# alexranaldi/CWSL_DIGI

Hardware: AMD Instinct MI355X
Metric: IQ Msamples/s demod+sync per GPU; concurrent FT8 slots at real-time; % HBM roofline (higher is better)
Workload: dtype f32

## Files before the change

cwsl_digi_amd/csrc/sync_host.inc:

```
namespace {

int sync_ensure_shared(cwslg_ctx *c)
{
    if (c->sync_shared.d_tables) return CWSLG_OK;
    constexpr double pi = 3.14159265358979323846;
    auto w = [&](int k, double n) { return make_float2((float)std::cos(2.0 * pi * k / n), (float)(-std::sin(2.0 * pi * k / n))); };
    auto half = [](float2 v) { return make_float2(0.5f * v.x, 0.5f * v.y); };
    auto same = [](float a, float b) { return std::memcmp(&a, &b, 4) == 0; };
    for (int k = 1; k <= 4; ++k)
        if (!same(w(k, 9.0).x, small_wr<9>(k)) || !same(w(k, 9.0).y, small_wi<9>(k)))
            return fail(c, CWSLG_ERR_HIP, "sync tables: W_9^%d computed on this host differs from the kernels' constants", k);
    for (int k = 1; k <= 2; ++k)
        if (!same(w(k, 5.0).x, w5_r(k)) || !same(w(k, 5.0).y, w5_i(k)))
            return fail(c, CWSLG_ERR_HIP, "sync tables: W_5^%d computed on this host differs from the kernels' constants", k);
    if (!same((float)(-std::sin(2.0 * pi / 3.0)), W3_S))
        return fail(c, CWSLG_ERR_HIP, "sync tables: sin(2 pi / 3) computed on this host differs from the kernels' constant");
    std::vector<float2> t;
    t.reserve(1920 + 64 + 1921 + 1152 + 1153);
    const float fac = 1.0f / 300.0f;
    for (int k = 0; k < 1920; ++k) { const float2 v = (k == 0) ? make_float2(1.f, 0.f) : w(k, 1920.0); t.push_back(make_float2(fac * v.x, fac * v.y)); }
    for (int k = 0; k < 64; ++k) t.push_back(w(k, 128.0));
    for (int k = 0; k <= 1920; ++k) t.push_back(half(k == 0 ? make_float2(1.f, 0.f) : w(k, 3840.0)));
    t[1920] = make_float2(1.f, 0.f); t[1920 + 32] = make_float2(0.f, -1.f);
    const size_t ft8_count = t.size();
    for (int k = 0; k < 1152; ++k) t.push_back(w(k, 1152.0));
    for (int k = 0; k <= 1152; ++k) t.push_back(half(k == 0 ? make_float2(1.f, 0.f) : w(k, 2304.0)));
    t[ft8_count] = make_float2(1.f, 0.f);
    HIPCHK(c, hipMalloc(&c->sync_shared.d_tables, t.size() * sizeof(float2)));
    HIPCHK(c, hipMemcpy(c->sync_shared.d_tables, t.data(), t.size() * sizeof(float2), hipMemcpyHostToDevice));
    c->sync_shared.t.w1920 = c->sync_shared.d_tables;
    c->sync_shared.t.w128 = c->sync_shared.d_tables + 1920;
    c->sync_shared.t.w3840 = c->sync_shared.d_tables + 1920 + 64;
    c->sync_shared.t.win = nullptr;
    float2 *t4 = c->sync_shared.d_tables + ft8_count;
    c->sync_shared.t4.w1920 = t4;
    c->sync_shared.t4.w128 = c->sync_shared.t.w128;
    c->sync_shared.t4.w3840 = t4 + 1152;
    std::vector<float> win(FT4_NFFT1);
    for (int i = 0; i < FT4_NFFT1; ++i)
        win[i] = (float)(0.3635819 - 0.4891775 * std::cos(2.0 * pi * i / 2304.0) + 0.1365995 * std::cos(4.0 * pi * i / 2304.0)
                         - 0.0106411 * std::cos(6.0 * pi * i / 2304.0));
    HIPCHK(c, hipMalloc(&c->sync_shared.d_win, win.size() * sizeof(float)));
    HIPCHK(c, hipMemcpy(c->sync_shared.d_win, win.data(), win.size() * sizeof(float), hipMemcpyHostToDevice));
    c->sync_shared.t4.win = c->sync_shared.d_win;
    return CWSLG_OK;
}

int ft4c_ensure_tables(cwslg_ctx *c)
{
    if (c->sync_shared.d_ft4c) return CWSLG_OK;
    constexpr double pi = 3.14159265358979323846;
    auto mk = [](double co, double si) { return make_float2((float)co, (float)si); };
    std::vector<float2> t;
    const size_t o567 = 0, on2 = o567 + F4C_NA, o2n = on2 + F4C_N2, o64 = o2n + F4C_N2 + 1, o63 = o64 + 32, o4032 = o63 + 63,
                 ocs = o4032 + F4C_NP, otw = ocs + 256, total = otw + 33 * 64;
    t.resize(total);
    for (int k = 0; k < F4C_NA; ++k) t[o567 + k] = mk(std::cos(2.0 * pi * k / 567.0), -std::sin(2.0 * pi * k / 567.0));
    for (int k = 0; k < F4C_N2; ++k) t[on2 + k] = mk(std::cos(2.0 * pi * k / 36288.0), -std::sin(2.0 * pi * k / 36288.0));
    for (int k = 0; k <= F4C_N2; ++k) t[o2n + k] = mk(std::cos(2.0 * pi * k / 72576.0), -std::sin(2.0 * pi * k / 72576.0));
    for (int k = 0; k < 32; ++k) t[o64 + k] = mk(std::cos(2.0 * pi * k / 64.0), -std::sin(2.0 * pi * k / 64.0));
    for (int k = 0; k < 63; ++k) t[o63 + k] = mk(std::cos(2.0 * pi * k / 63.0), -std::sin(2.0 * pi * k / 63.0));
    for (int k = 0; k < F4C_NP; ++k) t[o4032 + k] = mk(std::cos(2.0 * pi * k / 4032.0), -std::sin(2.0 * pi * k / 4032.0));
    t[o567] = t[on2] = t[o2n] = t[o64] = t[o63] = t[o4032] = mk(1.0, 0.0);
    t[o64 + 16] = mk(0.0, -1.0);
    {
        std::vector<float2> flat(t.begin() + on2, t.begin() + on2 + F4C_N2);
        for (int cc = 0; cc < F4C_NA; ++cc) for (int b = 0; b < 64; ++b) t[on2 + (size_t)cc * 64 + b] = flat[(size_t)b * cc];
        flat.assign(t.begin() + o4032, t.begin() + o4032 + F4C_NP);
        for (int cc = 0; cc < 63; ++cc) for (int b = 0; b < 64; ++b) t[o4032 + (size_t)cc * 64 + b] = flat[(size_t)b * cc];
    }
    static const int icos4[4][4] = {{0, 1, 3, 2}, {1, 0, 2, 3}, {2, 3, 1, 0}, {3, 2, 0, 1}};
    for (int b = 0; b < 4; ++b)
        for (int sy = 0; sy < 4; ++sy)
            for (int j = 0; j < 16; ++j) {
                const int p = (2 * icos4[b][sy] * j) % 32;
                float2 v = mk(std::cos(2.0 * pi * p / 32.0), std::sin(2.0 * pi * p / 32.0));
                if (p == 0) v = mk(1.0, 0.0);
                if (p == 8) v = mk(0.0, 1.0);
                if (p == 16) v = mk(-1.0, 0.0);
                if (p == 24) v = mk(0.0, -1.0);
                t[ocs + 64 * b + 16 * sy + j] = v;
            }
    for (int d = -16; d <= 16; ++d)
        for (int k = 0; k < 64; ++k) {
            const double a = 2.0 * pi * (double)d * (double)(k + 1) * 36.0 / 12000.0;
            t[otw + (d + 16) * 64 + k] = (d == 0) ? mk(1.0, 0.0) : mk(std::cos(a), std::sin(a));
        }
    std::vector<float> win(F4C_KHI - F4C_KLO + 1);
    for (int k = F4C_KLO; k <= F4C_KHI; ++k) {
        const int i = k + 126;
        double wv = 1.0;
        if (i < 63) wv = 0.5 * (1.0 + std::cos(pi * (double)(62 - i) / 63.0));
        else if (i >= 567) wv = 0.5 * (1.0 + std::cos(pi * (double)(i - 567) / 63.0));
        win[k - F4C_KLO] = (float)wv;
    }
    HIPCHK(c, hipMalloc(&c->sync_shared.d_ft4c, t.size() * sizeof(float2)));
    HIPCHK(c, hipMemcpy(c->sync_shared.d_ft4c, t.data(), t.size() * sizeof(float2), hipMemcpyHostToDevice));
    HIPCHK(c, hipMalloc(&c->sync_shared.d_ft4c_win, win.size() * sizeof(float)));
    HIPCHK(c, hipMemcpy(c->sync_shared.d_ft4c_win, win.data(), win.size() * sizeof(float), hipMemcpyHostToDevice));
    const float2 *b = c->sync_shared.d_ft4c;
    c->ft4_tables = Ft4Tables{b + o567, b + on2, b + o2n, b + o64, b + o63, b + o4032, b + ocs, b + otw, c->sync_shared.d_ft4c_win};
    return CWSLG_OK;
}

int ft4c_ensure_channel(cwslg_ctx *c, Channel &ch)
{
// ... 389 lines not shown
```

cwsl_digi_amd/csrc/sync_kernels.hpp:

```cpp
#pragma once
#include <hip/hip_runtime.h>
#include <stdint.h>

namespace cwslg {

constexpr int FT8_NSPS = 1920, FT8_NSTEP = 480, FT8_NHSYM = 372, FT8_NH1 = 1920, FT8_JZ = 62, FT8_NMAX = 180000;
constexpr int FT4_NFFT1 = 2304, FT4_NSTEP = 576, FT4_NHSYM = 122, FT4_NH1 = 1152, FT4_NMAX = 72576;
constexpr int FT4_ROW = 1168;
constexpr int SYNC_BAND = 32;
constexpr int SYNC_MAXCAND_CAP = 600;
constexpr int SYNC_MAXPRE = 1000;

struct SyncConfig {
    bool enabled = false;
    float syncmin = 1.5f;
    float syncmin_ft4 = 1.2f;
    bool ft4_coherent = true;
    int max_cand = 200;
    int order = 0;
    int f_lo_hz = 200, f_hi_hz = 3000;
    int ia = 64, ib = 960, nbins = 976;
};

struct SyncTables {
// ... 109 lines not shown
constexpr float W3_S = -0x1.bb67aep-1f;

template <int HALF>
__device__ __forceinline__ void stage1_pfa15(const float2 (&z)[8], float2 (*s_y)[SY_PITCH], const float2 *tw, int b)
{
    constexpr int KP = HALF ? 2 : 1;
    float2 Ya[3], Yb[3];
    {
        constexpr float w1r = w5r_at((1 * KP) % 5), w1i = w5i_at((1 * KP) % 5), w2r = w5r_at((2 * KP) % 5), w2i = w5i_at((2 * KP) % 5);
        float P = z[3].x * w1r, Q = z[3].y * w1i, R = z[3].x * w1i, S = z[3].y * w1r;
        P = __builtin_fmaf(z[6].x, w2r, P); Q = __builtin_fmaf(z[6].y, w2i, Q); R = __builtin_fmaf(z[6].x, w2i, R); S = __builtin_fmaf(z[6].y, w2r, S);
        Ya[0] = make_float2(z[0].x + (P - Q), z[0].y + (R + S));
        Yb[0] = make_float2(z[0].x + (P + Q), z[0].y + (S - R));
    }
    {
        constexpr float wr = w5r_at((4 * KP) % 5), wi = w5i_at((4 * KP) % 5);
        const float P = z[2].x * wr, Q = z[2].y * wi, R = z[2].x * wi, S = z[2].y * wr;
        Ya[1] = make_float2(z[5].x + (P - Q), z[5].y + (R + S));
        Yb[1] = make_float2(z[5].x + (P + Q), z[5].y + (S - R));
    }
    {
        constexpr float w1r = w5r_at((2 * KP) % 5), w1i = w5i_at((2 * KP) % 5), w2r = w5r_at((3 * KP) % 5), w2i = w5i_at((3 * KP) % 5),
                        w3r = w5r_at((4 * KP) % 5), w3i = w5i_at((4 * KP) % 5);
        float P = z[1].x * w1r, Q = z[1].y * w1i, R = z[1].x * w1i, S = z[1].y * w1r;
        P = __builtin_fmaf(z[4].x, w2r, P); Q = __builtin_fmaf(z[4].y, w2i, Q); R = __builtin_fmaf(z[4].x, w2i, R); S = __builtin_fmaf(z[4].y, w2r, S);
        P = __builtin_fmaf(z[7].x, w3r, P); Q = __builtin_fmaf(z[7].y, w3i, Q); R = __builtin_fmaf(z[7].x, w3i, R); S = __builtin_fmaf(z[7].y, w3r, S);
        Ya[2] = make_float2(P - Q, R + S);
        Yb[2] = make_float2(P + Q, S - R);
    }
    int n = 0;
    auto three = [&](const float2 y0, const float2 y1, const float2 y2, int k2) {
        const float2 x0 = make_float2((y0.x + y1.x) + y2.x, (y0.y + y1.y) + y2.y);
        const float2 t = make_float2(y1.x + y2.x, y1.y + y2.y), d = make_float2(y1.x - y2.x, y1.y - y2.y);
        const float2 m = make_float2(__builtin_fmaf(t.x, -0.5f, y0.x), __builtin_fmaf(t.y, -0.5f, y0.y));
        const float2 x1 = make_float2(__builtin_fmaf(-W3_S, d.y, m.x), __builtin_fmaf(W3_S, d.x, m.y));
        const float2 x2 = make_float2(__builtin_fmaf(W3_S, d.y, m.x), __builtin_fmaf(-W3_S, d.x, m.y));
        const int c0 = pfa15_c(0, k2), c1 = pfa15_c(1, k2), c2 = pfa15_c(2, k2);
        if (c0 == 0) s_y[0][b] = make_float2(x0.x * (1.0f / 300.0f), x0.y * (1.0f / 300.0f));
        else s_y[c0][b] = cmul_f(x0, tw[n++]);
        s_y[c1][b] = cmul_f(x1, tw[n++]);
        s_y[c2][b] = cmul_f(x2, tw[n++]);
    };
    if (HALF == 0) {
        const float2 d0 = make_float2((z[0].x + z[3].x) + z[6].x, (z[0].y + z[3].y) + z[6].y);
        const float2 d1 = make_float2(z[5].x + z[2].x, z[5].y + z[2].y);
        const float2 d2 = make_float2((z[1].x + z[4].x) + z[7].x, (z[1].y + z[4].y) + z[7].y);
        three(d0, d1, d2, 0);
    }
    three(Ya[0], Ya[1], Ya[2], KP);
    three(Yb[0], Yb[1], Yb[2], 5 - KP);
}

template <int HALF, int NA, int AMAX>
__device__ __forceinline__ void spectra_stage1_regs(const float2 (&z)[AMAX], float2 (*s_y)[SY_PITCH], const Stage1Tw<NA> &twp, int b);

template <int HALF, int NA, int NPACK>
__device__ __forceinline__ void spectra_stage1(const float *s_x, float2 (*s_y)[SY_PITCH], const Stage1Tw<NA> &twp, int b)
{
    constexpr int AMAX = (NPACK + 127) / 128;
    float2 z[AMAX];
#pragma unroll
    for (int a = 0; a < AMAX; ++a) {
        const int m = 128 * a + b;
        z[a] = (m < NPACK) ? make_float2(s_x[2 * m], s_x[2 * m + 1]) : make_float2(0.f, 0.f);
    }
    spectra_stage1_regs<HALF, NA, AMAX>(z, s_y, twp, b);
}

__device__ __forceinline__ void bfly(float2 &u, float2 &v, float2 w)
{
    const float ar = __builtin_fmaf(v.x, w.x, __builtin_fmaf(-v.y, w.y, u.x));
    const float ai = __builtin_fmaf(v.x, w.y, __builtin_fmaf(v.y, w.x, u.y));
    const float dr = __builtin_fmaf(2.0f, u.x, -ar);
    const float di = __builtin_fmaf(2.0f, u.y, -ai);
    u = make_float2(ar, ai);
    v = make_float2(dr, di);
}
__device__ __forceinline__ float unpack_power(float2 A, float2 B, float2 wh)
{
    B.y = -B.y;
    const float sr = A.x + B.x, si = A.y + B.y;
    const float2 o = make_float2(A.x - B.x, A.y - B.y);
    const float2 t = cmul_f(o, wh);
    const float xr = __builtin_fmaf(sr, 0.5f, t.y), xi = __builtin_fmaf(si, 0.5f, -t.x);
    return __builtin_fmaf(xr, xr, xi * xi);
}

__device__ __forceinline__ void bfly_one(float2 &u, float2 &v)
{
    const float2 a = make_float2(u.x + v.x, u.y + v.y);
    const float2 d = make_float2(u.x - v.x, u.y - v.y);
    u = a;
    v = d;
}
__device__ __forceinline__ void bfly_mj(float2 &u, float2 &v)
{
    const float2 a = make_float2(u.x + v.y, u.y - v.x);
    const float2 d = make_float2(u.x - v.y, u.y + v.x);
    u = a;
    v = d;
}

template <int NA, int NIN, int STEP, bool WINDOW>
__global__ __launch_bounds__(256) void symbol_spectra_kernel(const SyncWork *__restrict__ works, SyncTables tb, int nbins)
{
    constexpr int NZ = NA * 128;
    constexpr int NPACK = NIN / 2;
    constexpr int NGRP = NA * 16;
    static_assert(NGRP <= 256 && NIN % 8 == 0, "geometry");
    __shared__ float s_x[NIN];
    __shared__ float2 s_y[NA][SY_PITCH];
    __shared__ float2 s_w128[64];
    const SyncWork *w = works + blockIdx.y;
    const int j = blockIdx.x;
    const int tid = threadIdx.x;
    const int16_t *d = w->frame + (size_t)STEP * j;
    const float fac = 1.0f / 300.0f;
    Stage1Tw<NA> tw1;
    if (tid < 128) stage1_load_tw<0, NA>(tb.w1920, tid & 127, tw1);
    else stage1_load_tw<1, NA>(tb.w1920, tid & 127, tw1);
    constexpr int W3PRE = 4;
    float2 w3[W3PRE];
    const bool staged = nbins <= NIN;
    const int nfull = min(nbins, NZ) / (NA * 64);
#pragma unroll
    for (int i = 0; i < W3PRE; ++i) {
        const int it = (tid >> 6) + 4 * i;
        const int k = NA * (64 * (it / NA) + (tid & 63)) + it % NA;
        w3[i] = (staged && it < NA * nfull) ? tb.w3840[k] : make_float2(0.f, 0.f);
    }
    for (int t = tid; t < NIN / 8; t += 256) {
        const uint4 q = reinterpret_cast<const uint4 *>(d)[t];
        const unsigned v[4] = {q.x, q.y, q.z, q.w};
#pragma unroll
        for (int k = 0; k < 4; ++k) {
            float lo = (float)(short)(v[k] & 0xFFFFu), hi = (float)(short)(v[k] >> 16);
            if (NA != 15) { lo = fac * lo; hi = fac * hi; }
            if (WINDOW) { lo = lo * tb.win[8 * t + 2 * k]; hi = hi * tb.win[8 * t + 2 * k + 1]; }
            s_x[8 * t + 2 * k] = lo;
            s_x[8 * t + 2 * k + 1] = hi;
        }
    }
    if (tid >= 64 && tid < 128) s_w128[tid - 64] = tb.w128[tid - 64];
    __syncthreads();

    if (tid < 128) spectra_stage1<0, NA, NPACK>(s_x, s_y, tw1, tid & 127);
    else spectra_stage1<1, NA, NPACK>(s_x, s_y, tw1, tid & 127);
    __syncthreads();

    {
        const int c = tid >> 4, g = tid & 15;
        const int gb = (int)(__brev((unsigned)g) >> 28);
        float2 e[8];
        if (tid < NGRP) {
#pragma unroll
            for (int k = 0; k < 8; ++k) {
                const int k3 = ((k & 1) << 2) | (k & 2) | ((k >> 2) & 1);
                e[k] = s_y[c][16 * k3 + gb];
            }
        }
        __syncthreads();
        if (tid < NGRP) {
            bfly_one(e[0], e[1]); bfly_one(e[2], e[3]); bfly_one(e[4], e[5]); bfly_one(e[6], e[7]);
            bfly_one(e[0], e[2]); bfly_mj(e[1], e[3]); bfly_one(e[4], e[6]); bfly_mj(e[5], e[7]);
            bfly_one(e[0], e[4]); bfly(e[1], e[5], s_w128[16]); bfly_mj(e[2], e[6]); bfly(e[3], e[7], s_w128[48]);
#pragma unroll
// ... 27 lines not shown
        const int c = idx >> 6, k = idx & 63;
        float2 u = s_y[c][sy_col(k)], v = s_y[c][sy_col(k + 64)];
        bfly(u, v, s_w128[k]);
        s_y[c][sy_col(k)] = u;
        s_y[c][sy_col(k + 64)] = v;
    }
    __syncthreads();

    float *out = w->spectra + (size_t)j * nbins;
    auto power_at = [&](int k) -> float {
        const int k2 = (NZ - k) % NZ, kk = k % NZ;
        return unpack_power(s_y[kk % NA][sy_col(kk / NA)], s_y[k2 % NA][sy_col(k2 / NA)], tb.w3840[k]);
    };
    if (staged) {
        float *s_pw = s_x;
        const int lane = tid & 63, wv = tid >> 6;
        int pre = 0;
        for (int it = wv; it < NA * nfull; it += 4, ++pre) {
            const int r = it % NA, q = 64 * (it / NA) + lane;
            const int k = NA * q + r;
            const float2 A = s_y[r][sy_col(q)];
            const int r2 = (r == 0) ? 0 : NA - r;
            const int q2 = (r == 0) ? ((q == 0) ? 0 : 128 - q) : 127 - q;
            const float2 B = s_y[r2][sy_col(q2)];
            float2 wk;
            switch (pre) {
            case 0: wk = w3[0]; break;
            case 1: wk = w3[1]; break;
            case 2: wk = w3[2]; break;
            case 3: wk = w3[3]; break;
            default: wk = tb.w3840[k]; break;
            }
            s_pw[k] = unpack_power(A, B, wk);
        }
        for (int k = NA * 64 * nfull + tid; k < nbins; k += 256)
            s_pw[k] = (k <= NZ) ? power_at(k) : 0.0f;
        __syncthreads();
        for (int k = tid; k < nbins; k += 256) out[k] = s_pw[k];
    } else {
        for (int k = tid; k < nbins; k += 256) out[k] = (k <= NZ) ? power_at(k) : 0.0f;
    }
}

template <int HALF, int NA, int AMAX>
__device__ __forceinline__ void spectra_stage1_regs(const float2 (&z)[AMAX], float2 (*s_y)[SY_PITCH], const Stage1Tw<NA> &twp, int b)
{
    if constexpr (NA == 15) {
        static_assert(AMAX == 8, "FT8: 960 packed inputs = 8 rows of 128");
        stage1_pfa15<HALF>(z, s_y, twp.v, b);
    } else {
    constexpr int NPAIR = NA / 2, SPLIT = NPAIR / 2;
    constexpr int C0 = HALF ? SPLIT + 1 : 1, C1 = HALF ? NPAIR : SPLIT;
    const float2 *tw = twp.v;
    if (HALF == 0) {
        float2 s0 = z[0];
#pragma unroll
        for (int a = 1; a < AMAX; ++a) { s0.x = s0.x + z[a].x; s0.y = s0.y + z[a].y; }
        s_y[0][b] = s0;
    }
    float zero = 0.0f;
    asm volatile("" : "+v"(zero));
#pragma unroll
    for (int c = C0; c <= C1; ++c) {
        float P = zero, Q = zero, R = zero, S = zero;
#pragma unroll
        for (int a = 1; a < AMAX; ++a) {
            const int idx = (a * c) % NA;
            const float wr = small_wr<NA>((idx <= NA / 2) ? idx : NA - idx);
            const float wi = (idx <= NA / 2) ? small_wi<NA>(idx) : -small_wi<NA>(NA - idx);
            P = __builtin_fmaf(z[a].x, wr, P);
            Q = __builtin_fmaf(z[a].y, wi, Q);
            R = __builtin_fmaf(z[a].x, wi, R);
            S = __builtin_fmaf(z[a].y, wr, S);
        }
        const float2 yc = make_float2(z[0].x + (P - Q), z[0].y + (R + S));
        const float2 yn = make_float2(z[0].x + (P + Q), z[0].y + (S - R));
        s_y[c][b] = cmul_f(yc, tw[2 * (c - C0)]);
        s_y[NA - c][b] = cmul_f(yn, tw[2 * (c - C0) + 1]);
    }
    }
}

#ifndef CWSLG_SPEC_WAVES
#define CWSLG_SPEC_WAVES 4
#endif
#ifndef CWSLG_SPEC_HOISTPTR
#define CWSLG_SPEC_HOISTPTR 1
#endif
#ifndef CWSLG_SPEC_TIGHT
#define CWSLG_SPEC_TIGHT 1
#endif
#ifndef CWSLG_PLANE_NT
#define CWSLG_PLANE_NT 0
#endif
__device__ __forceinline__ void plane_store(CWSLG_GLOBAL v4f *p, v4f v)
{
    if (CWSLG_PLANE_NT & 1) __builtin_nontemporal_store(v, p); else *p = v;
}
__device__ __forceinline__ v4f plane_load4(const CWSLG_GLOBAL v4f *p)
{
    return (CWSLG_PLANE_NT & 2) ? __builtin_nontemporal_load(p) : *p;
}
__device__ __forceinline__ float plane_load1(const CWSLG_GLOBAL float *p)
{
    return (CWSLG_PLANE_NT & 2) ? __builtin_nontemporal_load(p) : *p;
}
inline int spectra_jper(int nsteps, size_t channels)
{
    for (int jper : {62, 31}) if (channels * (size_t)((nsteps + jper - 1) / jper) >= 3072) return jper;
    return 12;
}
#if defined(CWSLG_STAMP) && defined(CWSLG_STAMP_SPEC)
#define PSTAMP(slot)                                                                                                               \
    do {                                                                                                                           \
        const unsigned wg_ = blockIdx.y * gridDim.x + blockIdx.x;                                                                  \
        if (j == j0 + (jper >> 1) && (tid_ & 63) == 0 && wg_ < 16384) {                                                                     \
            unsigned long long t_;                                                                                                 \
            asm volatile("s_memtime %0\n\ts_waitcnt lgkmcnt(0)" : "=s"(t_)::"memory");                                             \
            g_stamps[32 * wg_ + 8 * (tid_ >> 6) + (slot)] = t_;                                                                    \
        }                                                                                                                          \
    } while (0)
#else
#define PSTAMP(slot) do { } while (0)
#endif
struct SpectraFin {
    const CWSLG_GLOBAL float *frame;
    CWSLG_GLOBAL int16_t *out;
    unsigned nv, s_end;
    float factor;
};
__device__ __forceinline__ unsigned fin_pack2(float x0, float x1, float factor)
{
    const float s0 = x0 * factor, s1 = x1 * factor;
    const float b0 = s0 + 0.5f, b1 = s1 + 0.5f;
    const int q0 = (int)b0, q1 = (int)b1;
    return ((unsigned)q0 & 0xFFFFu) | ((unsigned)q1 << 16);
}
__device__ __forceinline__ void spectra_finalize_range(const SpectraFin &F, unsigned s0, unsigned s1)
{
    typedef unsigned v4u __attribute__((ext_vector_type(4)));
    constexpr int NC = 4;
    for (unsigned base = s0 + threadIdx.x * 8u; base < s1; base += 256u * 8u * (unsigned)NC) {
        v4f a[NC], b[NC];
#pragma unroll
        for (int c = 0; c < NC; ++c) {
            const unsigned i0 = base + (unsigned)c * (256u * 8u);
            if (i0 + 8 <= F.nv && i0 < s1) {
                a[c] = *reinterpret_cast<const CWSLG_GLOBAL v4f *>(F.frame + i0);
                b[c] = *reinterpret_cast<const CWSLG_GLOBAL v4f *>(F.frame + i0 + 4);
            } else {
                float v[8];
#pragma unroll
                for (int k = 0; k < 8; ++k) v[k] = (i0 + k < F.nv && i0 < s1) ? F.frame[i0 + k] : 0.0f;
                a[c] = v4f{v[0], v[1], v[2], v[3]};
                b[c] = v4f{v[4], v[5], v[6], v[7]};
            }
        }
#pragma unroll
        for (int c = 0; c < NC; ++c) {
            const unsigned i0 = base + (unsigned)c * (256u * 8u);
            if (i0 >= s1) break;
            v4u pk;
            pk.x = fin_pack2(a[c].x, a[c].y, F.factor); pk.y = fin_pack2(a[c].z, a[c].w, F.factor);
            pk.z = fin_pack2(b[c].x, b[c].y, F.factor); pk.w = fin_pack2(b[c].z, b[c].w, F.factor);
            *reinterpret_cast<CWSLG_GLOBAL v4u *>(F.out + i0) = pk;
        }
    }
}

template <int NA, int NIN, int STEP, bool WINDOW, int FMODE = 0>
__global__ __launch_bounds__(256, CWSLG_SPEC_WAVES) void symbol_spectra_v2_kernel(const SyncWork *__restrict__ works, SyncTables tb, int nbins, int nsteps, int jper)
{
    static_assert(FMODE == 0 || (!WINDOW && NIN == 4 * STEP && STEP == 480), "the fused forms are FT8's");
    constexpr int NZ = NA * 128;
    constexpr int NPACK = NIN / 2;
    constexpr int NGRP = NA * 16;
    constexpr int AMAX = (NPACK + 127) / 128;
    constexpr int NH = NA / 2;
    constexpr int NITEM = (NH + 1) * 64, IPT = (NITEM + 255) / 256;
    static_assert(NGRP <= 256, "geometry");
    __shared__ __attribute__((aligned(16))) float s_pw[NIN + 32];
    __shared__ float2 s_y[NA][SY_PITCH];
    __shared__ float2 s_w128[64];
    constexpr int RING = NPACK + STEP / 2;
    __shared__ unsigned s_ring[FMODE == 2 ? 2 * RING : 1];
    const SyncWork *w = works + blockIdx.y;
    const int j0 = blockIdx.x * jper;
    const int jend = min(j0 + jper, nsteps);
    const int tid_ = threadIdx.x;
    const int b_ = tid_ & 127;
    const float fac = 1.0f / 300.0f;
    const CWSLG_GLOBAL unsigned *d32 = as_global(reinterpret_cast<const unsigned *>(w->frame)) + b_;
    float *const plane = w->spectra;
    const bool fuse = FMODE != 0;
    SpectraFin F{};
    v2f cv = {0.0f, 0.0f};
    unsigned fin_i = ~0u;
    unsigned fin_lim = 0u;
    constexpr int LOOK = 3;
    unsigned ring_rd = 0u, ring_wr = 0u;
    if (fuse) {
        const FinWork &f = w->fin;
        F.frame = as_global(f.frame); F.out = as_global_rw(f.out); F.nv = f.n_valid;
        const unsigned flen = f.frame_len;
        const float peak = __uint_as_float(*as_global(f.peak));
        float factor = 32767.0f / (peak + 1.0f);
        factor = factor * f.scale;
        F.factor = factor;
        if (blockIdx.x == 0 && tid_ == 0) {
            if (f.peak_next) *as_global_rw(f.peak_next) = 0u;
            if (f.factor_out) *as_global_rw(f.factor_out) = factor;
        }
        const unsigned cover = min((unsigned)(STEP * (nsteps - 1) + NIN), flen), tail_end = min(max(f.tail_end, cover), flen);
        if (tail_end > cover) {
            const unsigned per = ((tail_end - cover + gridDim.x - 1) / gridDim.x + 7u) & ~7u;
            spectra_finalize_range(F, min(cover + per * blockIdx.x, tail_end), min(cover + per * (blockIdx.x + 1), tail_end));
        }
        if constexpr (FMODE == 1) {
            F.s_end = min(((unsigned)(STEP * (jend - 1) + NIN) + 63u) & ~63u, flen);
            const unsigned e0 = min(((unsigned)(STEP * (j0 + LOOK - 1) + NIN) + 63u) & ~63u, F.s_end);
            spectra_finalize_range(F, (unsigned)(STEP * j0) & ~63u, e0);
            __builtin_amdgcn_s_waitcnt(0x0F70);
            __syncthreads();
            fin_lim = min(F.nv & ~1u, F.s_end);
            fin_i = e0 + 2u * (unsigned)tid_;
        } else {
            F.s_end = min((unsigned)(STEP * (jend - 1) + NIN), flen);
            fin_lim = min(F.nv & ~1u, F.s_end);
            const unsigned p0 = (unsigned)(STEP / 2) * (unsigned)j0;
            for (unsigned k = (unsigned)tid_; k < (unsigned)NPACK; k += 256u) {
                const unsigned i = 2u * (p0 + k);
                v2f p = {0.0f, 0.0f};
                if (i < fin_lim) p = *reinterpret_cast<const CWSLG_GLOBAL v2f *>(F.frame + i);
                const v2f bi = p * F.factor + 0.5f;
                const unsigned word = __builtin_amdgcn_perm((unsigned)(int)bi.y, (unsigned)(int)bi.x, 0x05040100u);
                if (i < F.s_end) *reinterpret_cast<CWSLG_GLOBAL unsigned *>(F.out + i) = word;
                const unsigned pos = (p0 + k) % (unsigned)RING;
                s_ring[pos] = word; s_ring[pos + RING] = word;
            }
            __syncthreads();
            fin_i = tid_ < STEP / 2 ? (unsigned)(STEP * j0 + NIN) + 2u * (unsigned)tid_ : 0x40000000u;
            ring_rd = (p0 + (unsigned)b_) % (unsigned)RING;
            ring_wr = (p0 + (unsigned)NPACK + (unsigned)tid_) % (unsigned)RING;
        }
        if (fin_i < fin_lim) cv = *reinterpret_cast<const CWSLG_GLOBAL v2f *>(F.frame + fin_i);
    }
    unsigned raw[AMAX];
    if constexpr (FMODE != 2) {
#pragma unroll
        for (int a = 0; a < AMAX; ++a) raw[a] = (128 * a + b_ < NPACK) ? d32[(STEP / 2) * j0 + 128 * a] : 0u;
    } else {
#pragma unroll
        for (int a = 0; a < AMAX; ++a) raw[a] = s_ring[ring_rd + 128 * a];
        ring_rd += (unsigned)(STEP / 2); if (ring_rd >= (unsigned)RING) ring_rd -= (unsigned)RING;
    }
    float2 wn[WINDOW ? AMAX : 1];
    if (WINDOW) {
#pragma unroll
        for (int a = 0; a < AMAX; ++a) {
            const int m = 128 * a + b_;
            wn[WINDOW ? a : 0] = *reinterpret_cast<const float2 *>(tb.win + 2 * ((m < NPACK) ? m : 0));
        }
    }
    Stage1Tw<NA> tw1;
    if (tid_ < 128) stage1_load_tw<0, NA>(tb.w1920, b_, tw1);
    else stage1_load_tw<1, NA>(tb.w1920, b_, tw1);
    const bool sparse = nbins >= NA * 64 && nbins <= NA * 64 + 32 && NH == 7;
    constexpr unsigned PW_DUMMY = 4u * (NIN + 31);
    float2 w3[IPT][2];
#ifndef CWSLG_SPEC_UNHOIST
#define CWSLG_SPEC_UNHOIST 0
#endif
    struct ItemAddr { unsigned au1[IPT], au2[IPT], aw1[IPT], aw2[IPT], ap1[IPT], ap2[IPT], aB[8]; bool iskip[IPT], izero[IPT]; };
    auto item_addr = [&](int tidx, ItemAddr &A, int (&K1o)[IPT], int (&K2o)[IPT]) {
#pragma unroll
    for (int i = 0; i < IPT; ++i) {
        const int it = tidx + 256 * i;
        int r = it >> 6, q = it & 63, kind = 0;
        bool skip = it >= NITEM || (r == 0 && q > 32);
        int Kup = 0;
        if (sparse && i == 0 && r == 0 && q > 32) {
            Kup = NA * 64 - 32 + q;
            const int d = Kup - NA * 64, a = d / NA, rem = d % NA;
            if (rem <= NH) { kind = 2; r = rem; q = a; }
            else { kind = 3; r = NA - rem; q = 63 - a; }
            skip = Kup >= nbins;
        }
        const int r2 = (r == 0) ? 0 : NA - r;
        const int k2 = (r == 0) ? ((64 - q) & 63) : 63 - q;
        A.izero[i] = r == 0 && q == 0 && kind == 0;
        if (sparse && A.izero[i]) kind = 1;
        A.iskip[i] = skip;
        const int rr = skip ? 0 : r, rr2 = skip ? 0 : r2;
        static_assert((SY_PITCH * 8) % 128 == 0, "row pitch");
        A.au1[i] = 8u * (unsigned)(rr * SY_PITCH + sy_col(q));
        A.au2[i] = 8u * (unsigned)(rr2 * SY_PITCH + sy_col(k2));
        A.aw1[i] = 8u * (unsigned)q; A.aw2[i] = 8u * (unsigned)k2;
        int K1 = NA * q + r, K2 = NA * k2 + r2;
        unsigned p1 = 4u * (unsigned)K1, p2 = 4u * (unsigned)K2;
        if (kind == 1) { K2 = NA * 64; p2 = (K2 < nbins) ? 4u * (unsigned)K2 : PW_DUMMY; }
        if (kind >= 2) { K1 = Kup; p1 = 4u * (unsigned)Kup; K2 = nbins; p2 = PW_DUMMY; }
        A.ap1[i] = p1 | ((unsigned)kind << 16); A.ap2[i] = p2;
        K1o[i] = (!skip && K1 < nbins) ? K1 : -1; K2o[i] = (!skip && K2 < nbins) ? K2 : -1;
    }
    {
        const int c = tidx >> 4, g = tidx & 15, blk = g >> 3, r = g & 7;
#pragma unroll
        for (int q = 0; q < 8; ++q) A.aB[q] = 8u * (unsigned)((tidx < NGRP ? c : 0) * SY_PITCH + sy_col(64 * blk + r + 8 * q));
    }
    };
    ItemAddr IA0;
    {
        int K1o[IPT], K2o[IPT];
        item_addr(tid_, IA0, K1o, K2o);
#pragma unroll
        for (int i = 0; i < IPT; ++i) {
            w3[i][0] = K1o[i] >= 0 ? tb.w3840[K1o[i]] : make_float2(0.f, 0.f);
            w3[i][1] = K2o[i] >= 0 ? tb.w3840[K2o[i]] : make_float2(0.f, 0.f);
        }
    }
    const bool wave0_ = __builtin_amdgcn_readfirstlane(tid_ >> 6) == 0;
    if (tid_ >= 64 && tid_ < 128) s_w128[tid_ - 64] = tb.w128[tid_ - 64];
    __builtin_amdgcn_s_waitcnt(0x0F70);

    for (int j = j0; j < jend; ++j) {
    int t = tid_;
    asm volatile("" : "+v"(t));
    const int tid = t, b = t & 127;
    ItemAddr IAj;
    int k1j[IPT], k2j[IPT];
    if (CWSLG_SPEC_UNHOIST) item_addr(tid, IAj, k1j, k2j);
    const ItemAddr &IA = CWSLG_SPEC_UNHOIST ? IAj : IA0;
    char *const sy_bytes = reinterpret_cast<char *>(&s_y[0][0]);
    const char *const w128_bytes = reinterpret_cast<const char *>(&s_w128[0]);
    char *const pw_bytes = reinterpret_cast<char *>(&s_pw[0]);
    PSTAMP(0);
    float2 z[AMAX];
#pragma unroll
    for (int a = 0; a < AMAX; ++a) {
        const bool live = 128 * a + b < NPACK;
        float lo = (float)(short)(raw[a] & 0xFFFFu), hi = (float)(short)(raw[a] >> 16);
        if (NA != 15) { lo = fac * lo; hi = fac * hi; }
        if (WINDOW) { lo = lo * wn[WINDOW ? a : 0].x; hi = hi * wn[WINDOW ? a : 0].y; }
        z[a] = live ? make_float2(lo, hi) : make_float2(0.f, 0.f);
    }
#ifndef CWSLG_SPEC_LOADS_FIRST
#define CWSLG_SPEC_LOADS_FIRST 0
#endif
#ifndef CWSLG_FUSE_STORE_NT
#define CWSLG_FUSE_STORE_NT 0
#endif
    auto store_prev_row = [&]() {
#ifdef CWSLG_SPEC_DIAG_NOSTORE
        if (j > j0 && nbins < 0) {
#else
        if (j > j0) {
#endif
            CWSLG_GLOBAL v4f *out4 = reinterpret_cast<CWSLG_GLOBAL v4f *>(as_global_rw(CWSLG_SPEC_HOISTPTR ? plane : w->spectra) + (size_t)(j - 1) * nbins);
            if (NA == 15) { if (tid >= 128) for (int k4 = tid - 128; 4 * k4 < nbins; k4 += 128) plane_store(out4 + k4, *reinterpret_cast<const v4f *>(s_pw + 4 * k4)); }
            else for (int k4 = tid; 4 * k4 < nbins; k4 += 256) plane_store(out4 + k4, *reinterpret_cast<const v4f *>(s_pw + 4 * k4));
        }
    };
    if (!CWSLG_SPEC_LOADS_FIRST) store_prev_row();
    if (fuse) {
        const v2f sc = cv * F.factor;
        const v2f bi = sc + 0.5f;
        const int q0 = (int)bi.x, q1 = (int)bi.y;
        const unsigned word = __builtin_amdgcn_perm((unsigned)q1, (unsigned)q0, 0x05040100u);
        if (fin_i < F.s_end) {
            if (CWSLG_FUSE_STORE_NT) __builtin_nontemporal_store(word, reinterpret_cast<CWSLG_GLOBAL unsigned *>(F.out + fin_i));
            else *reinterpret_cast<CWSLG_GLOBAL unsigned *>(F.out + fin_i) = word;
            if constexpr (FMODE == 2) { s_ring[ring_wr] = word; s_ring[ring_wr + RING] = word; }
        }
        if constexpr (FMODE == 2) {
            fin_i += (unsigned)STEP;
            ring_wr += (unsigned)(STEP / 2); if (ring_wr >= (unsigned)RING) ring_wr -= (unsigned)RING;
        } else {
            fin_i += 512u;
        }
        cv = v2f{0.0f, 0.0f};
        if (fin_i < fin_lim) cv = *reinterpret_cast<const CWSLG_GLOBAL v2f *>(F.frame + fin_i);
    }
    {
        const int jn = CWSLG_SPEC_TIGHT ? min(j + 1, jend - 1) : j + 1;
        if constexpr (FMODE != 2) {
        if (CWSLG_SPEC_TIGHT || j + 1 < jend)
#pragma unroll
        for (int a = 0; a < AMAX; ++a) raw[a] = (128 * a + b < NPACK) ? d32[(STEP / 2) * jn + 128 * a] : 0u;
        }
    }
    if (CWSLG_SPEC_LOADS_FIRST) store_prev_row();

    if (tid < 128) spectra_stage1_regs<0, NA, AMAX>(z, s_y, tw1, b);
    else spectra_stage1_regs<1, NA, AMAX>(z, s_y, tw1, b);
    PSTAMP(1);
    lds_barrier();
    PSTAMP(2);
    if constexpr (FMODE == 2) {
#pragma unroll
        for (int a = 0; a < AMAX; ++a) raw[a] = s_ring[ring_rd + 128 * a];
        ring_rd += (unsigned)(STEP / 2); if (ring_rd >= (unsigned)RING) ring_rd -= (unsigned)RING;
    }

#ifndef CWSLG_SPEC_MERGE_AB
#define CWSLG_SPEC_MERGE_AB 1
#endif
    const bool inAB = tid < NGRP;
    if (CWSLG_SPEC_MERGE_AB ? inAB : true) {
    {
        const int c = tid >> 4, g = tid & 15;
        const int gb = (int)(__brev((unsigned)g) >> 28);
        float2 e[8];
        if (CWSLG_SPEC_MERGE_AB || inAB) {
            const char *const pa = sy_bytes + 8u * (unsigned)(c * SY_PITCH + gb);
#pragma unroll
            for (int k = 0; k < 8; ++k) {
                const int k3 = ((k & 1) << 2) | (k & 2) | ((k >> 2) & 1);
                e[k] = CWSLG_SPEC_TIGHT ? *reinterpret_cast<const float2 *>(pa + 128 * k3) : s_y[c][16 * k3 + gb];
            }
        }
        __builtin_amdgcn_fence(__ATOMIC_RELEASE, "wavefront");
        __builtin_amdgcn_wave_barrier();
        __builtin_amdgcn_fence(__ATOMIC_ACQUIRE, "wavefront");
        if (CWSLG_SPEC_MERGE_AB || inAB) {
            bfly_one(e[0], e[1]); bfly_one(e[2], e[3]); bfly_one(e[4], e[5]); bfly_one(e[6], e[7]);
            bfly_one(e[0], e[2]); bfly_mj(e[1], e[3]); bfly_one(e[4], e[6]); bfly_mj(e[5], e[7]);
            bfly_one(e[0], e[4]); bfly(e[1], e[5], s_w128[16]); bfly_mj(e[2], e[6]); bfly(e[3], e[7], s_w128[48]);
            const unsigned a0 = 8u * (unsigned)(c * SY_PITCH + sy_col(8 * g));
#pragma unroll
            for (int k = 0; k < 8; ++k) {
                if (CWSLG_SPEC_TIGHT) *reinterpret_cast<float2 *>(sy_bytes + (a0 ^ (8u * k))) = e[k];
                else s_y[c][sy_col(8 * g + k)] = e[k];
            }
        }
    }
    __builtin_amdgcn_fence(__ATOMIC_RELEASE, "wavefront");
    __builtin_amdgcn_wave_barrier();
    __builtin_amdgcn_fence(__ATOMIC_ACQUIRE, "wavefront");
    PSTAMP(3);
    if (CWSLG_SPEC_MERGE_AB || inAB) {
        const int r = tid & 7;
        float2 e[8];
#pragma unroll
        for (int q = 0; q < 8; ++q) e[q] = *reinterpret_cast<const float2 *>(sy_bytes + IA.aB[q]);
        {
            const float2 w0 = s_w128[r * 8];
            bfly(e[0], e[1], w0); bfly(e[2], e[3], w0); bfly(e[4], e[5], w0); bfly(e[6], e[7], w0);
        }
        {
            const float2 w0 = s_w128[r * 4], w1 = s_w128[(r + 8) * 4];
            bfly(e[0], e[2], w0); bfly(e[1], e[3], w1); bfly(e[4], e[6], w0); bfly(e[5], e[7], w1);
        }
        {
            bfly(e[0], e[4], s_w128[r * 2]); bfly(e[1], e[5], s_w128[(r + 8) * 2]);
            bfly(e[2], e[6], s_w128[(r + 16) * 2]); bfly(e[3], e[7], s_w128[(r + 24) * 2]);
        }
#pragma unroll
        for (int q = 0; q < 8; ++q) *reinterpret_cast<float2 *>(sy_bytes + IA.aB[q]) = e[q];
    }
    }
    PSTAMP(4);
    lds_barrier();
    PSTAMP(5);

    float2 w3j[IPT][2];
    if (CWSLG_SPEC_UNHOIST) {
#pragma unroll
        for (int i = 0; i < IPT; ++i) {
            w3j[i][0] = k1j[i] >= 0 ? tb.w3840[k1j[i]] : make_float2(0.f, 0.f);
            w3j[i][1] = k2j[i] >= 0 ? tb.w3840[k2j[i]] : make_float2(0.f, 0.f);
        }
    }
    const float2 (&w3u)[IPT][2] = CWSLG_SPEC_UNHOIST ? w3j : w3;
#pragma unroll
    for (int i = 0; i < IPT; ++i) {
        if (IA.iskip[i]) continue;
        float2 u1 = *reinterpret_cast<const float2 *>(sy_bytes + IA.au1[i]), v1 = *reinterpret_cast<const float2 *>(sy_bytes + (IA.au1[i] ^ 64u) + 512);
        float2 u2 = *reinterpret_cast<const float2 *>(sy_bytes + IA.au2[i]), v2 = *reinterpret_cast<const float2 *>(sy_bytes + (IA.au2[i] ^ 64u) + 512);
        bfly(u1, v1, *reinterpret_cast<const float2 *>(w128_bytes + IA.aw1[i]));
        bfly(u2, v2, *reinterpret_cast<const float2 *>(w128_bytes + IA.aw2[i]));
        if (sparse) {
            float2 A1 = u1, B1 = v2, A2 = u2;
            unsigned p1 = IA.ap1[i];
            if (i == 0 && wave0_) {
                const unsigned kind = p1 >> 16;
                p1 &= 0xFFFFu;
                A1 = (kind == 2) ? v1 : (kind == 3) ? v2 : u1;
                B1 = (kind == 0) ? v2 : (kind == 2) ? u2 : u1;
                A2 = (kind == 1) ? v1 : u2;
            }
            *reinterpret_cast<float *>(pw_bytes + p1) = unpack_power(A1, B1, w3u[i][0]);
            *reinterpret_cast<float *>(pw_bytes + IA.ap2[i]) = unpack_power(A2, v1, w3u[i][1]);
            continue;
        }
        if (IA.izero[i]) {
            s_pw[0] = unpack_power(u1, u1, w3u[i][0]);
            if (NA * 64 < nbins) s_pw[NA * 64] = unpack_power(v1, v1, tb.w3840[NA * 64]);
            if (NZ < nbins) s_pw[NZ] = unpack_power(u1, u1, tb.w3840[NZ]);
            continue;
        }
        const int K1 = (int)(IA.ap1[i] >> 2), K2 = (int)(IA.ap2[i] >> 2);
        const int K3 = K1 + NA * 64, K4 = K2 + NA * 64;
        if (K1 < nbins) s_pw[K1] = unpack_power(u1, v2, w3u[i][0]);
        if (K2 < nbins) s_pw[K2] = unpack_power(u2, v1, w3u[i][1]);
        if (K3 < nbins) s_pw[K3] = unpack_power(v1, u2, tb.w3840[K3]);
        if (K4 < nbins) s_pw[K4] = unpack_power(v2, u1, tb.w3840[K4]);
    }
    for (int k = NZ + 1 + tid; k < nbins; k += 256) s_pw[k] = 0.0f;
    PSTAMP(6);
    lds_barrier();
    PSTAMP(7);
    }
    if (jend > j0) {
        CWSLG_GLOBAL v4f *out4 = reinterpret_cast<CWSLG_GLOBAL v4f *>(as_global_rw(w->spectra) + (size_t)(jend - 1) * nbins);
        for (int k4 = tid_; 4 * k4 < nbins; k4 += 256) plane_store(out4 + k4, *reinterpret_cast<const v4f *>(s_pw + 4 * k4));
    }
}

constexpr int SYNC2D_NT = 512;
__device__ __forceinline__ unsigned long long sync_key(float v, int l)
{
    unsigned u = __float_as_uint(v);
    u = (u & 0x80000000u) ? ~u : (u | 0x80000000u);
    return ((unsigned long long)u << 32) | (unsigned)(255 - l);
}
template <int CTRL>
__device__ __forceinline__ unsigned long long dpp_u64(unsigned long long k)
{
    const int lo = __builtin_amdgcn_update_dpp((int)(unsigned)k, (int)(unsigned)k, CTRL, 0xf, 0xf, false);
    const int hi = __builtin_amdgcn_update_dpp((int)(unsigned)(k >> 32), (int)(unsigned)(k >> 32), CTRL, 0xf, 0xf, false);
    return ((unsigned long long)(unsigned)hi << 32) | (unsigned)lo;
}
__device__ __forceinline__ unsigned long long wave_max_u64(unsigned long long k)
{
    unsigned long long o;
    o = dpp_u64<0xB1>(k); k = (o > k) ? o : k;
    o = dpp_u64<0x4E>(k); k = (o > k) ? o : k;
    o = dpp_u64<0x141>(k); k = (o > k) ? o : k;
    o = dpp_u64<0x140>(k); k = (o > k) ? o : k;
#pragma unroll
    for (int msk = 16; msk <= 32; msk <<= 1) {
        const unsigned lo = __shfl_xor((unsigned)k, msk, 64);
        const unsigned hi = __shfl_xor((unsigned)(k >> 32), msk, 64);
        o = ((unsigned long long)hi << 32) | lo;
        k = (o > k) ? o : k;
    }
    return k;
}
__device__ __forceinline__ float key_value(unsigned long long k)
{
    unsigned u = (unsigned)(k >> 32);
    u = (u & 0x80000000u) ? (u & 0x7FFFFFFFu) : ~u;
    return __uint_as_float(u);
}

#if CWSLG_LAB
struct SyncPair { float a, b; };
__device__ __forceinline__ SyncPair costas_sync2(const float (*s_s)[376], const float *s_c0, int rr, int j)
{
    const int icos[7] = {3, 1, 4, 0, 6, 5, 2};
    float ta0 = 0, tb0 = 0, tc0 = 0, ua0 = 0, ub0 = 0, uc0 = 0;
    float ta1 = 0, tb1 = 0, tc1 = 0, ua1 = 0, ub1 = 0, uc1 = 0;
#pragma unroll
    for (int n = 0; n < 7; ++n) {
        const int m = j + 12 + 4 * n;
        const float *row = s_s[rr + 2 * icos[n]];
        {
            const int mc = (m < 0) ? 0 : m;
            const float2 v = *reinterpret_cast<const float2 *>(row + mc), c = *reinterpret_cast<const float2 *>(s_c0 + mc);
            const bool ok0 = m >= 1, ok1 = m + 1 >= 1;
            ta0 = ta0 + (ok0 ? v.x : 0.0f); ua0 = ua0 + (ok0 ? c.x : 0.0f);
            ta1 = ta1 + (ok1 ? v.y : 0.0f); ua1 = ua1 + (ok1 ? c.y : 0.0f);
        }
        {
            const float2 v = *reinterpret_cast<const float2 *>(row + m + 144), c = *reinterpret_cast<const float2 *>(s_c0 + m + 144);
            tb0 = tb0 + v.x; ub0 = ub0 + c.x;
            tb1 = tb1 + v.y; ub1 = ub1 + c.y;
        }
        {
            const int mm = m + 288, mc = (mm > 374) ? 374 : mm;
            const float2 v = *reinterpret_cast<const float2 *>(row + mc), c = *reinterpret_cast<const float2 *>(s_c0 + mc);
            const bool ok0 = mm <= FT8_NHSYM, ok1 = mm + 1 <= FT8_NHSYM;
            tc0 = tc0 + (ok0 ? v.x : 0.0f); uc0 = uc0 + (ok0 ? c.x : 0.0f);
            tc1 = tc1 + (ok1 ? v.y : 0.0f); uc1 = uc1 + (ok1 ? c.y : 0.0f);
        }
    }
    auto finish = [](float ta, float tb, float tc, float t0a, float t0b, float t0c) {
// ... 976 lines not shown
```

Baseline: 317,700.

## Derive mirrored FT8 spectra addresses and twiddles to cut registers, raise occupancy

For the NA==15 FT8 spectra kernel, some LDS addresses and one twiddle per item are now computed from others. The stage-B addresses come from aB[0] via XOR, and the second item's address, weight and power index come from the first via subtraction. The K2 twiddle is taken as a mirror of K1's W_3840 value, with a host check that confirms the symmetry bit-exactly. Fewer hoisted values should free VGPRs, so launch bounds for the fused FT8 variant are raised from 4 to 5 waves. A forced waitcnt is added and the UNHOIST debug path is removed, at the cost of extra ALU ops and inline asm that blocks some compiler scheduling.

```diff
diff --git a/cwsl_digi_amd/csrc/sync_host.inc b/cwsl_digi_amd/csrc/sync_host.inc
--- a/cwsl_digi_amd/csrc/sync_host.inc
+++ b/cwsl_digi_amd/csrc/sync_host.inc
@@ -22,6 +22,11 @@
     for (int k = 0; k < 64; ++k) t.push_back(w(k, 128.0));
     for (int k = 0; k <= 1920; ++k) t.push_back(half(k == 0 ? make_float2(1.f, 0.f) : w(k, 3840.0)));
     t[1920] = make_float2(1.f, 0.f); t[1920 + 32] = make_float2(0.f, -1.f);
+    for (int k = 1; k < 960; ++k) {
+        const float2 a = t[1920 + 64 + k], m = t[1920 + 64 + 960 - k];
+        if (!same(m.x, -a.y) || !same(m.y, -a.x))
+            return fail(c, CWSLG_ERR_HIP, "sync tables: W_3840^%d is not the mirror image of W_3840^%d on this host", 960 - k, k);
+    }
     const size_t ft8_count = t.size();
     for (int k = 0; k < 1152; ++k) t.push_back(w(k, 1152.0));
     for (int k = 0; k <= 1152; ++k) t.push_back(half(k == 0 ? make_float2(1.f, 0.f) : w(k, 2304.0)));
diff --git a/cwsl_digi_amd/csrc/sync_kernels.hpp b/cwsl_digi_amd/csrc/sync_kernels.hpp
--- a/cwsl_digi_amd/csrc/sync_kernels.hpp
+++ b/cwsl_digi_amd/csrc/sync_kernels.hpp
@@ -215,6 +215,16 @@
     const float sr = A.x + B.x, si = A.y + B.y;
     const float2 o = make_float2(A.x - B.x, A.y - B.y);
     const float2 t = cmul_f(o, wh);
+    const float xr = __builtin_fmaf(sr, 0.5f, t.y), xi = __builtin_fmaf(si, 0.5f, -t.x);
+    return __builtin_fmaf(xr, xr, xi * xi);
+}
+
+__device__ __forceinline__ float unpack_power_mirror(float2 A, float2 B, float2 wk)
+{
+    B.y = -B.y;
+    const float sr = A.x + B.x, si = A.y + B.y;
+    const float2 o = make_float2(A.x - B.x, A.y - B.y);
+    const float2 t = make_float2(__builtin_fmaf(-o.x, wk.y, o.y * wk.x), __builtin_fmaf(-o.x, wk.x, -(o.y * wk.y)));
     const float xr = __builtin_fmaf(sr, 0.5f, t.y), xi = __builtin_fmaf(si, 0.5f, -t.x);
     return __builtin_fmaf(xr, xr, xi * xi);
 }
@@ -408,8 +418,20 @@
 }
 
 #ifndef CWSLG_SPEC_WAVES
-#define CWSLG_SPEC_WAVES 4
+#define CWSLG_SPEC_WAVES 5
 #endif
+template <unsigned K> __device__ __forceinline__ unsigned spec_xor_k(unsigned x)
+{
+    unsigned r;
+    asm volatile("v_xor_b32 %0, %1, %2" : "=v"(r) : "n"(K), "v"(x));
+    return r;
+}
+template <unsigned K> __device__ __forceinline__ unsigned spec_rsub_k(unsigned x)
+{
+    unsigned r;
+    asm volatile("v_sub_u32 %0, %1, %2" : "=v"(r) : "n"(K), "v"(x));
+    return r;
+}
 #ifndef CWSLG_SPEC_HOISTPTR
 #define CWSLG_SPEC_HOISTPTR 1
 #endif
@@ -495,7 +517,7 @@
 }
 
 template <int NA, int NIN, int STEP, bool WINDOW, int FMODE = 0>
-__global__ __launch_bounds__(256, CWSLG_SPEC_WAVES) void symbol_spectra_v2_kernel(const SyncWork *__restrict__ works, SyncTables tb, int nbins, int nsteps, int jper)
+__global__ __launch_bounds__(256, (NA == 15 && FMODE == 1) ? CWSLG_SPEC_WAVES : 4) void symbol_spectra_v2_kernel(const SyncWork *__restrict__ works, SyncTables tb, int nbins, int nsteps, int jper)
 {
     static_assert(FMODE == 0 || (!WINDOW && NIN == 4 * STEP && STEP == 480), "the fused forms are FT8's");
     constexpr int NZ = NA * 128;
@@ -593,10 +615,8 @@
     else stage1_load_tw<1, NA>(tb.w1920, b_, tw1);
     const bool sparse = nbins >= NA * 64 && nbins <= NA * 64 + 32 && NH == 7;
     constexpr unsigned PW_DUMMY = 4u * (NIN + 31);
+    constexpr bool DERIVE = NA == 15;
     float2 w3[IPT][2];
-#ifndef CWSLG_SPEC_UNHOIST
-#define CWSLG_SPEC_UNHOIST 0
-#endif
     struct ItemAddr { unsigned au1[IPT], au2[IPT], aw1[IPT], aw2[IPT], ap1[IPT], ap2[IPT], aB[8]; bool iskip[IPT], izero[IPT]; };
     auto item_addr = [&](int tidx, ItemAddr &A, int (&K1o)[IPT], int (&K2o)[IPT]) {
 #pragma unroll
@@ -644,6 +664,7 @@
             w3[i][0] = K1o[i] >= 0 ? tb.w3840[K1o[i]] : make_float2(0.f, 0.f);
             w3[i][1] = K2o[i] >= 0 ? tb.w3840[K2o[i]] : make_float2(0.f, 0.f);
         }
+        if (DERIVE) w3[1][0] = tb.w3840[IA0.ap1[1] >> 2];
     }
     const bool wave0_ = __builtin_amdgcn_readfirstlane(tid_ >> 6) == 0;
     if (tid_ >= 64 && tid_ < 128) s_w128[tid_ - 64] = tb.w128[tid_ - 64];
@@ -653,10 +674,8 @@
     int t = tid_;
     asm volatile("" : "+v"(t));
     const int tid = t, b = t & 127;
-    ItemAddr IAj;
-    int k1j[IPT], k2j[IPT];
-    if (CWSLG_SPEC_UNHOIST) item_addr(tid, IAj, k1j, k2j);
-    const ItemAddr &IA = CWSLG_SPEC_UNHOIST ? IAj : IA0;
+    if constexpr (FMODE == 1) __builtin_amdgcn_s_waitcnt(0x0F70);
+    const ItemAddr &IA = IA0;
     char *const sy_bytes = reinterpret_cast<char *>(&s_y[0][0]);
     const char *const w128_bytes = reinterpret_cast<const char *>(&s_w128[0]);
     char *const pw_bytes = reinterpret_cast<char *>(&s_pw[0]);
@@ -767,8 +786,16 @@
     if (CWSLG_SPEC_MERGE_AB || inAB) {
         const int r = tid & 7;
         float2 e[8];
-#pragma unroll
-        for (int q = 0; q < 8; ++q) e[q] = *reinterpret_cast<const float2 *>(sy_bytes + IA.aB[q]);
+        unsigned aBq[8];
+#pragma unroll
+        for (int q = 0; q < 8; ++q) aBq[q] = IA.aB[q];
+        if (DERIVE) {
+            aBq[1] = spec_xor_k<8 | 64>(IA.aB[0]); aBq[2] = spec_xor_k<16>(IA.aB[0]); aBq[3] = spec_xor_k<24 | 64>(IA.aB[0]); aBq[4] = spec_xor_k<32>(IA.aB[0]);
+            aBq[5] = spec_xor_k<40 | 64>(IA.aB[0]); aBq[6] = spec_xor_k<48>(IA.aB[0]); aBq[7] = spec_xor_k<56 | 64>(IA.aB[0]);
+        }
+        constexpr int BOFF = DERIVE ? 64 : 0;
+#pragma unroll
+        for (int q = 0; q < 8; ++q) e[q] = *reinterpret_cast<const float2 *>(sy_bytes + aBq[q] + BOFF * (q & ~1));
         {
             const float2 w0 = s_w128[r * 8];
             bfly(e[0], e[1], w0); bfly(e[2], e[3], w0); bfly(e[4], e[5], w0); bfly(e[6], e[7], w0);
@@ -782,29 +809,28 @@
             bfly(e[2], e[6], s_w128[(r + 16) * 2]); bfly(e[3], e[7], s_w128[(r + 24) * 2]);
         }
 #pragma unroll
-        for (int q = 0; q < 8; ++q) *reinterpret_cast<float2 *>(sy_bytes + IA.aB[q]) = e[q];
+        for (int q = 0; q < 8; ++q) *reinterpret_cast<float2 *>(sy_bytes + aBq[q] + BOFF * (q & ~1)) = e[q];
     }
     }
     PSTAMP(4);
     lds_barrier();
     PSTAMP(5);
 
-    float2 w3j[IPT][2];
-    if (CWSLG_SPEC_UNHOIST) {
-#pragma unroll
-        for (int i = 0; i < IPT; ++i) {
-            w3j[i][0] = k1j[i] >= 0 ? tb.w3840[k1j[i]] : make_float2(0.f, 0.f);
-            w3j[i][1] = k2j[i] >= 0 ? tb.w3840[k2j[i]] : make_float2(0.f, 0.f);
-        }
-    }
-    const float2 (&w3u)[IPT][2] = CWSLG_SPEC_UNHOIST ? w3j : w3;
+    const float2 (&w3u)[IPT][2] = w3;
 #pragma unroll
     for (int i = 0; i < IPT; ++i) {
         if (IA.iskip[i]) continue;
+        const bool drv = DERIVE && i == 1;
+        unsigned au2 = IA.au2[i], aw2 = IA.aw2[i], ap2 = IA.ap2[i];
+        if (drv) {
+            au2 = spec_xor_k<56>(spec_rsub_k<8 * (NA * SY_PITCH) + 504>(IA.au1[i]));
+            aw2 = spec_rsub_k<8 * 63>(IA.aw1[i]);
+            ap2 = spec_rsub_k<4 * (NA * 64)>(IA.ap1[i]);
+        }
         float2 u1 = *reinterpret_cast<const float2 *>(sy_bytes + IA.au1[i]), v1 = *reinterpret_cast<const float2 *>(sy_bytes + (IA.au1[i] ^ 64u) + 512);
-        float2 u2 = *reinterpret_cast<const float2 *>(sy_bytes + IA.au2[i]), v2 = *reinterpret_cast<const float2 *>(sy_bytes + (IA.au2[i] ^ 64u) + 512);
+        float2 u2 = *reinterpret_cast<const float2 *>(sy_bytes + au2), v2 = *reinterpret_cast<const float2 *>(sy_bytes + (au2 ^ 64u) + 512);
         bfly(u1, v1, *reinterpret_cast<const float2 *>(w128_bytes + IA.aw1[i]));
-        bfly(u2, v2, *reinterpret_cast<const float2 *>(w128_bytes + IA.aw2[i]));
+        bfly(u2, v2, *reinterpret_cast<const float2 *>(w128_bytes + aw2));
         if (sparse) {
             float2 A1 = u1, B1 = v2, A2 = u2;
             unsigned p1 = IA.ap1[i];
@@ -816,7 +842,7 @@
                 A2 = (kind == 1) ? v1 : u2;
             }
             *reinterpret_cast<float *>(pw_bytes + p1) = unpack_power(A1, B1, w3u[i][0]);
-            *reinterpret_cast<float *>(pw_bytes + IA.ap2[i]) = unpack_power(A2, v1, w3u[i][1]);
+            *reinterpret_cast<float *>(pw_bytes + ap2) = drv ? unpack_power_mirror(A2, v1, w3u[i][0]) : unpack_power(A2, v1, w3u[i][1]);
             continue;
         }
         if (IA.izero[i]) {
@@ -825,10 +851,10 @@
             if (NZ < nbins) s_pw[NZ] = unpack_power(u1, u1, tb.w3840[NZ]);
             continue;
         }
-        const int K1 = (int)(IA.ap1[i] >> 2), K2 = (int)(IA.ap2[i] >> 2);
+        const int K1 = (int)(IA.ap1[i] >> 2), K2 = (int)(ap2 >> 2);
         const int K3 = K1 + NA * 64, K4 = K2 + NA * 64;
         if (K1 < nbins) s_pw[K1] = unpack_power(u1, v2, w3u[i][0]);
-        if (K2 < nbins) s_pw[K2] = unpack_power(u2, v1, w3u[i][1]);
+        if (K2 < nbins) s_pw[K2] = drv ? unpack_power_mirror(u2, v1, w3u[i][0]) : unpack_power(u2, v1, w3u[i][1]);
         if (K3 < nbins) s_pw[K3] = unpack_power(v1, u2, tb.w3840[K3]);
         if (K4 < nbins) s_pw[K4] = unpack_power(v2, u1, tb.w3840[K4]);
     }
```

New measurement: 318,400, median of 3. About the same (+0.2%).
